# pyprob/pyprob

Measured on NVIDIA H100. Metric: ic_train_traces_per_sec, higher is better.
Workload: dtype f32

## Files before the change

pyprob_b200/csrc/net.cu:

```cuda
#include <vector>
#include <string.h>
#include <stdlib.h>
#include <stdint.h>

#include "common.cuh"
#include "gemm_simt.cuh"
#include "heads.cuh"
#include "tc_grouped.cuh"
#include "tc_lstm.cuh"
#include "tc_cluster.cuh"
#include "tc_persist.cuh"
#include "obs_mlp.cuh"

using gemm::Problem;

struct HImg {
  float* k_hi = nullptr; float* k_lo = nullptr; float* mn_hi = nullptr; float* mn_lo = nullptr;
  int64_t kb = 0;
};

struct WImg {
  int64_t k_hi = 0, k_lo = 0, mn_hi = 0, mn_lo = 0;
  int kb = 0;
};
struct PackEntry {
  int64_t src_off;
  int rows, cols, ld, kb;
  int64_t k_hi, k_lo, mn_hi, mn_lo;
  int tile_start, pad_;
};

enum class ObsForm { fused, tensor_core, simt };

struct ppb_net {
  float* wimg = nullptr;
  int64_t wimg_floats = 0;
  std::vector<PackEntry> pack;
  PackEntry* d_pack = nullptr;
  int pack_tiles = 0;
  WImg w_ihE, w_hh;
  std::vector<WImg> w1, w2;
  ObsForm obs_form = ObsForm::simt;
  WImg w_obs[PPB_MAX_OBS][PPB_MAX_FF_LAYERS];
  WImg w_fin[PPB_MAX_FF_LAYERS];
  uint64_t slot_hash[10] = {0, 0, 0, 0, 0, 0, 0, 0, 0, 0};
  const void* slot_dev[10] = {nullptr, nullptr, nullptr, nullptr, nullptr, nullptr, nullptr, nullptr, nullptr, nullptr};
  void* h_blob[2] = {nullptr, nullptr};
  cudaEvent_t ev_blob[2] = {nullptr, nullptr};
  size_t blob_cap = 0;
  int blob_idx = 0;
  ppb_net_desc desc;
  std::vector<ppb_addr_desc> addrs;
  std::vector<int64_t> type_off;
  ppb_addr_desc* d_addrs = nullptr;
  int64_t* d_type_off = nullptr;
  int64_t arena_floats = 0;
  int I = 0;
  int dh_pad = 4;
  int out_pad = 4;
  bool fused_cell = true;
  float* whh_il = nullptr;
  int64_t whh_il_floats = 0;
  void* d_lstm_steps = nullptr;
  size_t lstm_steps_cap = 0;
  cudaStream_t side[2] = {nullptr, nullptr};
  cudaEvent_t fork_ev[16] = {nullptr, nullptr, nullptr, nullptr, nullptr, nullptr, nullptr, nullptr,
                             nullptr, nullptr, nullptr, nullptr, nullptr, nullptr, nullptr, nullptr};
  int fork_next = 0;
  int single_stream = 0;
  int pack_tiles_no_hh = 0;
  int host_graph = 1;
  cudaStream_t host_stream = nullptr;
  cudaGraphExec_t host_exec = nullptr;
  uint64_t host_key = 0;
  int host_seen = 0;
  float* host_hyper_dev = nullptr;
  void* host_state_dev = nullptr;
  float host_hyper[6] = {0, 0, 0, 0, 0, 0};
  int64_t host_step_dev = -1;
  char* host_pin = nullptr;
  int64_t host_pin_cap = 0;
  Problem* h_stage[2] = {nullptr, nullptr};
  cudaEvent_t ev_stage[2] = {nullptr, nullptr};
  size_t stage_cap = 0;
  int stage_idx = 0;
};

namespace {

inline int64_t align_up(int64_t x, int64_t a) { return (x + a - 1) / a * a; }

struct Ws {
  float* obs_act[PPB_MAX_OBS][PPB_MAX_FF_LAYERS];
  float* obs_cat; float* fin_act[PPB_MAX_FF_LAYERS]; float* obs_emb;
  float* p_obs; float* emb_cat; float* p_step; float* w_smp_t; float* smp_emb;
  float* gates; float* c; float* h; float* hid; float* out_raw; float* row_lp; float* d_out;
  float* loss_acc;
  float* d_hid; float* dh; float* dh_rec; float* dc; float* d_pobs; float* d_pstep; float* d_smp; float* d_embcat;
  float* d_obs_emb; float* d_fin_act[PPB_MAX_FF_LAYERS]; float* d_obs_cat; float* d_obs_act[PPB_MAX_OBS][PPB_MAX_FF_LAYERS];
  Problem* problems;
  int64_t max_problems;
  int64_t total_bytes;
};

struct Dims {
  int B, R, T, NS, G;
};

Ws carve(const ppb_net* net, Dims d, void* base) {
  const ppb_net_desc& D = net->desc;
  Ws w;
  memset(&w, 0, sizeof(w));
  char* p = (char*)base;
  int64_t off = 0;
  auto take = [&](int64_t floats) {
    float* r = (float*)(p + off);
    off += align_up(floats * 4, 256);
    return r;
  };
  const int H = D.lstm_dim, E = D.obs_dim, S = D.sample_dim, C2 = 2 * (D.type_dim + D.addr_dim);
  for (int j = 0; j < D.num_obs; ++j)
    for (int l = 0; l + 1 < D.obs_ff[j].num_layers; ++l) w.obs_act[j][l] = take((int64_t)d.B * D.obs_ff[j].layers[l].out_dim);
  w.obs_cat = take((int64_t)d.B * E);
  for (int l = 0; l + 1 < D.obs_final.num_layers; ++l) w.fin_act[l] = take((int64_t)d.B * D.obs_final.layers[l].out_dim);
  w.obs_emb = take((int64_t)d.B * E);
  w.p_obs = take((int64_t)d.B * 4 * H);
  w.emb_cat = take((int64_t)d.NS * C2);
  w.p_step = take((int64_t)d.NS * 4 * H);
  w.w_smp_t = take((int64_t)S * 4 * H);
  w.smp_emb = take((int64_t)d.R * S);
  w.gates = take((int64_t)d.R * 4 * H);
  w.c = take((int64_t)d.R * H);
  w.h = take((int64_t)d.R * H);
  w.hid = take((int64_t)d.R * net->dh_pad);
  w.out_raw = take((int64_t)d.R * net->out_pad);
  w.row_lp = take(d.R);
  w.d_out = take((int64_t)d.R * net->out_pad);
  w.loss_acc = take(64);
  w.d_hid = take((int64_t)d.R * net->dh_pad);
  w.dh = take((int64_t)d.R * H);
  w.dh_rec = take((int64_t)d.R * H);
  w.dc = take((int64_t)d.R * H);
  w.d_pobs = take((int64_t)d.B * 4 * H);
  w.d_smp = take((int64_t)d.R * S);
  w.d_embcat = take((int64_t)d.NS * C2);
  w.d_pstep = take((int64_t)d.NS * 4 * H);
  w.d_obs_emb = take((int64_t)d.B * E);
  for (int l = 0; l + 1 < D.obs_final.num_layers; ++l) w.d_fin_act[l] = take((int64_t)d.B * D.obs_final.layers[l].out_dim);
  w.d_obs_cat = take((int64_t)d.B * E);
  for (int j = 0; j < D.num_obs; ++j)
    for (int l = 0; l + 1 < D.obs_ff[j].num_layers; ++l) w.d_obs_act[j][l] = take((int64_t)d.B * D.obs_ff[j].layers[l].out_dim);
  w.max_problems = 2 * (64 + 4LL * PPB_MAX_OBS * PPB_MAX_FF_LAYERS + 8LL * d.G + 4LL * d.T);
  w.problems = (Problem*)take(w.max_problems * (int64_t)(sizeof(Problem) / 4));
  w.total_bytes = off;
  return w;
}

inline float* dgates_ptr(const Ws& w, void* base) { return (float*)((char*)base + w.total_bytes); }
inline int64_t dgates_bytes(const ppb_net* net, Dims d) { return align_up((int64_t)d.R * 4 * net->desc.lstm_dim * 4, 256); }

struct Builder {
  std::vector<Problem> probs;
  std::vector<gemm::Phase> phases;
  void begin() { gemm::Phase ph; ph.first = (int)probs.size(); phases.push_back(ph); }
  void add(Problem p) {
    gemm::Phase& ph = phases.back();
    p.tiles_m = (p.M + gemm::BM - 1) / gemm::BM;
    p.tiles_n = (p.N + gemm::BN - 1) / gemm::BN;
    p.tile_start = ph.tiles;
    if (p.M <= 0 || p.N <= 0) return;
    ph.tiles += p.tiles_m * p.tiles_n;
    ph.count += 1;
    probs.push_back(p);
  }
};

inline Problem P0() {
  Problem p;
  memset(&p, 0, sizeof(p));
  p.alpha = 1.0f;
  return p;
}

inline Problem linear_fwd(const float* X, int64_t ldx, const float* W, int64_t ldw, const float* b, float* Y,
                          int64_t ldy, int M, int N, int K, int flags) {
  Problem p = P0();
  p.A = X; p.sam = ldx; p.sak = 1;
  p.B = W; p.sbn = ldw; p.sbk = 1;
  p.C = Y; p.ldc = ldy; p.bias = b;
  p.M = M; p.N = N; p.K = K; p.flags = flags;
  return p;
}
inline Problem linear_dx(const float* dY, int64_t lddy, const float* W, int64_t ldw, float* dX, int64_t lddx, int M,
                         int N, int K, int flags) {
  Problem p = P0();
  p.A = dY; p.sam = lddy; p.sak = 1;
  p.B = W; p.sbn = 1; p.sbk = ldw;
  p.C = dX; p.ldc = lddx;
  p.M = M; p.N = K; p.K = N; p.flags = flags;
  return p;
}
inline Problem linear_dw(const float* dY, int64_t lddy, const float* X, int64_t ldx, float* dW, int64_t ldw, int M,
                         int N, int K) {
  Problem p = P0();
  p.A = dY; p.sam = 1; p.sak = lddy;
  p.B = X; p.sbn = 1; p.sbk = ldx;
  p.C = dW; p.ldc = ldw;
  p.M = N; p.N = K; p.K = M; p.flags = gemm::kAccumulate;
  return p;
}

inline uint64_t fnv1a(const void* data, size_t n, uint64_t h = 1469598103934665603ULL) {
  const unsigned char* p = (const unsigned char*)data;
  for (size_t i = 0; i < n; ++i) { h ^= p[i]; h *= 1099511628211ULL; }
  return h;
}

int upload_cached(ppb_net* net, int slot, const void* src, size_t bytes, void* dev, cudaStream_t st) {
  if (bytes == 0) return PPB_OK;
  uint64_t h = fnv1a(src, bytes, 1469598103934665603ULL ^ (uint64_t)bytes);
  if (net->slot_hash[slot] == h && net->slot_dev[slot] == dev) return PPB_OK;
// ... 384 lines not shown
  NllArgs A;
  float* loss_acc; float* loss_out; int* status_out;
  struct State { float local; int bad; };
  using RowIn = NllRowIn;
  __device__ __forceinline__ RowIn load(int64_t row) const { return nll_row_in(A, (int)row); }
  __device__ __forceinline__ void row(State& s, const RowIn& in, const float* x, int64_t row, int lane) const {
    nll_row(A, in, x, (int)row, lane, s.local, s.bad);
  }
  __device__ __forceinline__ void finish(const State& s, int lane) const {
    nll_finish(s.local, s.bad, lane, A.inv_batch, gridDim.x, loss_acc, loss_out, status_out);
  }
};

__global__ void __launch_bounds__(256) k_head_nll(const float* __restrict__ out_raw, NllArgs A, int R,
                                                   float* __restrict__ loss_acc, float* __restrict__ loss_out,
                                                   int* __restrict__ status_out) {
  ppb_pdl_trigger();
  ppb_pdl_wait();
  const int lane = threadIdx.x & 31;
  const int warp = (blockIdx.x * blockDim.x + threadIdx.x) >> 5, nwarps = (gridDim.x * blockDim.x) >> 5;
  float local = 0.0f;
  int bad = 0;
  for (int row = warp; row < R; row += nwarps) nll_row(A, out_raw + (int64_t)row * A.out_pad, row, lane, local, bad);
  nll_finish(local, bad, lane, A.inv_batch, gridDim.x, loss_acc, loss_out, status_out);
}

__global__ void __launch_bounds__(256, 4) k_head_out_nll(const float* __restrict__ arena, const float* __restrict__ hid_hi,
                                                       const float* __restrict__ hid_lo, int64_t hid_kb,
                                                       const int* __restrict__ step_row0, const int* __restrict__ step_nrows,
                                                       int rows_per_block, NllArgs A, float* __restrict__ out_raw,
                                                       float* __restrict__ loss_acc, float* __restrict__ loss_out,
                                                       int* __restrict__ status_out) {
  ppb_pdl_trigger();
  extern __shared__ float sm_head[];
  const int seg = blockIdx.y, warp = threadIdx.x >> 5, lane = threadIdx.x & 31;
  const ppb_addr_desc a = A.addrs[A.step_addr[seg]];
  const int Hh = a.head_hidden, O = a.head_out, Hh4 = (Hh + 3) & ~3;
  const int pitch = ((Hh4 >> 2) & 1) ? Hh4 : Hh4 + 4;
  float* w2s = sm_head;
  float* b2s = w2s + (size_t)O * pitch;
  float* hrow = b2s + ((O + 3) & ~3) + (size_t)warp * (Hh4 + 128);
  float* xout = hrow + Hh4;
  const int r0 = step_row0[seg] + blockIdx.x * rows_per_block;
  int r1 = r0 + rows_per_block;
  const int seg_end = step_row0[seg] + step_nrows[seg];
  const int seg_end_pad = step_row0[seg] + ((step_nrows[seg] + 127) & ~127);
  if (r1 > seg_end_pad) r1 = seg_end_pad;
  const bool any = r0 < r1 && r0 < seg_end;
  if (any) {
    const float* w2 = arena + a.w2_off;
    for (int i = threadIdx.x; i < O * pitch; i += blockDim.x) {
      const int o = i / pitch, k = i - o * pitch;
      w2s[i] = (k < Hh) ? __ldg(w2 + (int64_t)o * Hh + k) : 0.0f;
    }
    for (int o = threadIdx.x; o < O; o += blockDim.x) b2s[o] = __ldg(arena + a.b2_off + o);
  }
  ppb_pdl_wait();
  __syncthreads();
  float local = 0.0f;
  int bad = 0;
  for (int row = r0 + warp; row < r1; row += 8) {
    if (row >= seg_end) {
      nll_row(A, xout, row, lane, local, bad);
      continue;
    }
    for (int k = lane; k < Hh4; k += 32) {
      float v = 0.0f;
      if (k < Hh) {
        const int64_t off = tc::packed_offset(row, k, hid_kb);
        v = __ldg(hid_hi + off) + (hid_lo ? __ldg(hid_lo + off) : 0.0f);
      }
      hrow[k] = v;
    }
    __syncwarp();
    for (int o0 = 0; o0 < O; o0 += 32) {
      const int o = o0 + lane;
      const float4* wr = reinterpret_cast<const float4*>(w2s + (size_t)(o < O ? o : 0) * pitch);
      const float4* hr = reinterpret_cast<const float4*>(hrow);
      float acc[4] = {0.f, 0.f, 0.f, 0.f};
#pragma unroll 4
      for (int k4 = 0; k4 < (Hh4 >> 2); ++k4) {
        const float4 h4 = hr[k4], w4 = wr[k4];
        acc[0] = fmaf(h4.x, w4.x, acc[0]);
        acc[1] = fmaf(h4.y, w4.y, acc[1]);
        acc[2] = fmaf(h4.z, w4.z, acc[2]);
        acc[3] = fmaf(h4.w, w4.w, acc[3]);
      }
      if (o < O) {
        const float y = ((acc[0] + acc[1]) + (acc[2] + acc[3])) + b2s[o];
        xout[o] = y;
        if (out_raw) out_raw[(int64_t)row * A.out_pad + o] = y;
      }
    }
    __syncwarp();
    nll_row(A, xout, row, lane, local, bad);
    __syncwarp();
  }
  nll_finish(local, bad, lane, A.inv_batch, gridDim.x * gridDim.y, loss_acc, loss_out, status_out);
}

__device__ __forceinline__ float cell_bwd_unit(float ig, float fg, float gg, float og, float cn, float cp, float dht,
                                               float dc_next, float (&dv)[4]) {
  const float tc_ = ppb_cell_tanh(cn);
  const float dct = dc_next + dht * og * (1.0f - tc_ * tc_);
  dv[0] = dct * gg * ig * (1.0f - ig);
  dv[1] = dct * cp * fg * (1.0f - fg);
  dv[2] = dct * ig * (1.0f - gg * gg);
  dv[3] = dht * tc_ * og * (1.0f - og);
  return dct;
}

__device__ __forceinline__ void img_store_gates(const HImg& img, int64_t row, int j, int64_t gate_stride, const float (&v)[4]) {
  const int64_t ok = tc::packed_offset(row, j, img.kb), omn = tc::packed_offset_mn(row, j, img.kb);
#pragma unroll
  for (int q = 0; q < 4; ++q) {
    float hi, lo;
    tc::split_tf32(v[q], hi, lo);
    img.k_hi[ok + q * gate_stride] = hi;
    if (img.k_lo) img.k_lo[ok + q * gate_stride] = lo;
    if (img.mn_hi) {
      img.mn_hi[omn + q * gate_stride] = hi;
      if (img.mn_lo) img.mn_lo[omn + q * gate_stride] = lo;
    }
  }
}

struct CellBwdT1Epi {
  const float* gates; const float* c; const int* row_trace;
  float* dgates; HImg pimg; int H;
  __device__ __forceinline__ void cells(int64_t row, int j0, const float (&dh)[4]) const {
    const int tr = __ldg(row_trace + row);
    const int64_t gate_stride = (int64_t)(H >> 5) * tc::kTileFloats;
    float gv[4][4], cv[4];
#pragma unroll
    for (int u = 0; u < 4; ++u) {
      const int j = min(j0 + 32 * u, H - 1);
#pragma unroll
      for (int q = 0; q < 4; ++q) gv[u][q] = __ldg(gates + row * 4 * H + q * H + j);
      cv[u] = __ldg(c + row * H + j);
    }
#pragma unroll
    for (int u = 0; u < 4; ++u) {
      const int j = j0 + 32 * u;
      if (j >= H) continue;
      float dv[4] = {0.f, 0.f, 0.f, 0.f};
      if (tr >= 0) cell_bwd_unit(gv[u][0], gv[u][1], gv[u][2], gv[u][3], cv[u], 0.0f, dh[u], 0.0f, dv);
#pragma unroll
      for (int q = 0; q < 4; ++q) dgates[row * 4 * H + q * H + j] = dv[q];
      if (tr >= 0) img_store_gates(pimg, tr, j, gate_stride, dv);
    }
  }
};

template <bool FINAL>
__global__ void __launch_bounds__(256, FINAL ? 4 : 8) k_cell_bwd(const float* __restrict__ gates, const float* __restrict__ c,
                                                   const float* __restrict__ dh, const float* __restrict__ dh_rec,
                                                   float* __restrict__ dc, float* __restrict__ dgates,
                                                   float* __restrict__ d_pobs, const int* __restrict__ row_prev,
                                                   const int* __restrict__ row_next, const int* __restrict__ row_trace,
                                                   HImg gimg, int row0, int n_rows, int H, int t, HImg pimg) {
  ppb_pdl_trigger();
  ppb_pdl_wait();
  const int64_t total = (int64_t)n_rows * H;
  const int64_t gate_stride = (int64_t)(H >> 5) * tc::kTileFloats;
  const bool h32 = (H & 31) == 0;
  for (int64_t e = (int64_t)blockIdx.x * blockDim.x + threadIdx.x; e < total; e += (int64_t)gridDim.x * blockDim.x) {
    const int i = (int)(e / H), j = (int)(e - (int64_t)i * H);
    const int row = row0 + i;
    const int tr = __ldg(row_trace + row);
    const int64_t rH = (int64_t)row * H + j;
    float* dgr = dgates + (int64_t)row * 4 * H + j;
    float dv[4] = {0.f, 0.f, 0.f, 0.f};
    if (tr >= 0) {
      const int nx = __ldg(row_next + row);
      const float* g = gates + (int64_t)row * 4 * H + j;
      const float ig = g[0], fg = g[H], gg = g[2 * H], og = g[3 * H];
      const float cn = c[rH];
      const float cp = (t > 0) ? c[(int64_t)__ldg(row_prev + row) * H + j] : 0.0f;
      const bool has_next = nx >= 0;
      const float dht = dh[rH] + (has_next ? dh_rec[rH] : 0.0f);
      const float dct = cell_bwd_unit(ig, fg, gg, og, cn, cp, dht, has_next ? dc[(int64_t)nx * H + j] : 0.0f, dv);
      if (dc) dc[rH] = dct * fg;
      float* dp = d_pobs + (int64_t)tr * 4 * H + j;
      float tot[4];
#pragma unroll
      for (int q = 0; q < 4; ++q) {
        tot[q] = has_next ? dp[q * H] + dv[q] : dv[q];
        dp[q * H] = tot[q];
      }
      if (FINAL && pimg.k_hi) img_store_gates(pimg, tr, j, gate_stride, tot);
    }
#pragma unroll
    for (int q = 0; q < 4; ++q) dgr[q * H] = dv[q];
    if (gimg.k_hi) {
      if (h32) {
        img_store_gates(gimg, row, j, gate_stride, dv);
      } else {
#pragma unroll
        for (int q = 0; q < 4; ++q)
          tcg::img_store(gimg.k_hi, gimg.k_lo, gimg.mn_hi, gimg.mn_lo, row, q * H + j, gimg.kb, dv[q]);
      }
    }
  }
}

__global__ void __launch_bounds__(256) k_step_colsum(const float* __restrict__ dgates, const int* __restrict__ step_row0,
                                                      const int* __restrict__ step_nrows, int H4,
                                                      float* __restrict__ d_pstep) {
  __shared__ float part[8][33];
  const int st = blockIdx.y;
  const int r0 = step_row0[st], n = step_nrows[st];
  const int lane = threadIdx.x & 31, slice = threadIdx.x >> 5;
  const int col = blockIdx.x * 32 + lane;
  float s = 0.0f;
  if (col < H4)
    for (int r = slice; r < n; r += 8) s += dgates[(int64_t)(r0 + r) * H4 + col];
  part[slice][lane] = s;
  __syncthreads();
  if (slice == 0 && col < H4) {
    float t = 0.0f;
#pragma unroll
    for (int k = 0; k < 8; ++k) t += part[k][lane];
    d_pstep[(int64_t)st * H4 + col] = t;
  }
}

__global__ void __launch_bounds__(128) k_smp_bwd(const float* __restrict__ dgates, const float* __restrict__ w_smp_t,
                                                  const float* __restrict__ smp_emb, const float* __restrict__ values,
                                                  const int* __restrict__ row_step, const int* __restrict__ step_prev,
                                                  const int* __restrict__ row_prev,
                                                  const ppb_addr_desc* __restrict__ addrs, int R, int H4, int S,
                                                  float* __restrict__ grad) {
  int warp = (blockIdx.x * blockDim.x + threadIdx.x) >> 5, lane = threadIdx.x & 31;
  int nwarps = (gridDim.x * blockDim.x) >> 5;
  for (int row = warp; row < R; row += nwarps) {
    int pa = step_prev[row_step[row]];
    if (pa < 0) continue;
    const ppb_addr_desc& a = addrs[pa];
    float x = values[row_prev[row]];
    for (int j = 0; j < S; ++j) {
      float s = 0.0f;
      for (int col = lane; col < H4; col += 32) s = fmaf(dgates[(int64_t)row * H4 + col], w_smp_t[(int64_t)j * H4 + col], s);
      s = ppb_warp_sum(s);
      if (lane == 0 && smp_emb[(int64_t)row * S + j] > 0.0f && s != 0.0f) {
        atomicAdd(grad + a.smp_b_off + j, s);
        if (a.family == PPB_FAMILY_CATEGORICAL) {
          int cidx = (int)x;
          if (cidx >= 0 && cidx < a.smp_in) atomicAdd(grad + a.smp_w_off + (int64_t)j * a.smp_in + cidx, s);
        } else {
          atomicAdd(grad + a.smp_w_off + (int64_t)j * a.smp_in, s * x);
        }
      }
    }
  }
}

__global__ void __launch_bounds__(128) k_smp_bwd_seg(const float* __restrict__ dgates, const float* __restrict__ w_smp_t,
                                                      const float* __restrict__ smp_emb, const float* __restrict__ values,
                                                      const int* __restrict__ step_prev, const int* __restrict__ step_row0,
                                                      const int* __restrict__ step_nrows, const int* __restrict__ row_prev,
                                                      const ppb_addr_desc* __restrict__ addrs, int H4, int S,
                                                      int rows_per_block, float* __restrict__ grad) {
  __shared__ float acc_b[8];
  __shared__ float acc_w[8][heads::CMAX];
  const int st = blockIdx.y;
  const int pa = step_prev[st];
  if (pa < 0) return;
  const int seg0 = step_row0[st], r0 = seg0 + blockIdx.x * rows_per_block;
  int r1 = r0 + rows_per_block;
  if (r1 > seg0 + step_nrows[st]) r1 = seg0 + step_nrows[st];
  if (r0 >= r1) return;
  const ppb_addr_desc a = addrs[pa];
  const bool is_cat = a.family == PPB_FAMILY_CATEGORICAL;
  const int width = is_cat ? a.smp_in : 1;
  for (int i = threadIdx.x; i < 8 * heads::CMAX; i += blockDim.x) (&acc_w[0][0])[i] = 0.0f;
  if (threadIdx.x < 8) acc_b[threadIdx.x] = 0.0f;
  __syncthreads();
  const int warp = threadIdx.x >> 5, lane = threadIdx.x & 31;
  for (int row = r0 + warp; row < r1; row += 4) {
    float s[8];
#pragma unroll
    for (int j = 0; j < 8; ++j) s[j] = 0.0f;
    for (int col = lane; col < H4; col += 32) {
      const float d = dgates[(int64_t)row * H4 + col];
#pragma unroll
      for (int j = 0; j < 8; ++j)
        if (j < S) s[j] = fmaf(d, __ldg(w_smp_t + (int64_t)j * H4 + col), s[j]);
    }
#pragma unroll
    for (int j = 0; j < 8; ++j)
      if (j < S) s[j] = ppb_warp_sum(s[j]);
    if (lane == 0) {
      const float x = values[row_prev[row]];
      const int cidx = (int)x;
#pragma unroll
      for (int j = 0; j < 8; ++j) {
        if (j < S && smp_emb[(int64_t)row * S + j] > 0.0f && s[j] != 0.0f) {
          atomicAdd(&acc_b[j], s[j]);
          if (is_cat) { if (cidx >= 0 && cidx < a.smp_in) atomicAdd(&acc_w[j][cidx], s[j]); }
          else atomicAdd(&acc_w[j][0], s[j] * x);
        }
      }
    }
  }
  __syncthreads();
  for (int i = threadIdx.x; i < S * (width + 1); i += blockDim.x) {
// ... 130 lines not shown
    }
    for (int j = 0; j < S; ++j)
      if (acc[j] != 0.0f) atomicAdd(dw_ih + (int64_t)col * I + E + j, acc[j]);
  }
}

__global__ void k_bias_grad(const float* __restrict__ d_pstep, int NS, int H4, float* __restrict__ db_ih,
                            float* __restrict__ db_hh) {
  for (int col = blockIdx.x * blockDim.x + threadIdx.x; col < H4; col += gridDim.x * blockDim.x) {
    float s = 0.0f;
    for (int st = 0; st < NS; ++st) s += d_pstep[(int64_t)st * H4 + col];
    db_ih[col] += s;
    db_hh[col] += s;
  }
}
__global__ void k_embed_scatter(const float* __restrict__ d_embcat, const ppb_addr_desc* __restrict__ addrs,
                                const int64_t* __restrict__ type_off, const int* __restrict__ step_addr,
                                const int* __restrict__ step_prev, int n_steps, int td, int ad,
                                float* __restrict__ grad) {
  int C2 = 2 * (td + ad);
  for (int64_t e = (int64_t)blockIdx.x * blockDim.x + threadIdx.x; e < (int64_t)n_steps * C2;
       e += (int64_t)gridDim.x * blockDim.x) {
    int st = (int)(e / C2), j = (int)(e % C2);
    int which = j < (td + ad) ? step_prev[st] : step_addr[st];
    int jj = j < (td + ad) ? j : j - (td + ad);
    if (which < 0) continue;
    const ppb_addr_desc& a = addrs[which];
    float v = d_embcat[e];
    if (v == 0.0f) continue;
    if (jj < td) atomicAdd(grad + type_off[a.type_id] + jj, v);
    else atomicAdd(grad + a.addr_emb_off + (jj - td), v);
  }
}
__global__ void __launch_bounds__(256) k_colsum_gather(const float* __restrict__ dY, int64_t ld,
                                                        const int* __restrict__ m_gather, int M, int N,
                                                        float* __restrict__ db) {
  __shared__ float part[8][33];
  const int lane = threadIdx.x & 31, slice = threadIdx.x >> 5;
  const int n = blockIdx.x * 32 + lane;
  float s = 0.0f;
  if (n < N)
    for (int m = blockIdx.y * 8 + slice; m < M; m += 8 * gridDim.y) {
      int64_t pm = m_gather ? m_gather[m] : m;
      s += dY[pm * ld + n];
    }
  part[slice][lane] = s;
  __syncthreads();
  if (slice == 0 && n < N) {
    float t = 0.0f;
#pragma unroll
    for (int k = 0; k < 8; ++k) t += part[k][lane];
    if (t != 0.0f) atomicAdd(db + n, t);
  }
}
__global__ void k_scale(float* __restrict__ x, int64_t n, float a) {
  for (int64_t i = (int64_t)blockIdx.x * blockDim.x + threadIdx.x; i < n; i += (int64_t)gridDim.x * blockDim.x) x[i] *= a;
}

__global__ void k_add_row_bias(float* __restrict__ p, const float* __restrict__ b, int64_t n, int H4) {
  for (int64_t i = (int64_t)blockIdx.x * blockDim.x + threadIdx.x; i < n; i += (int64_t)gridDim.x * blockDim.x) p[i] += b[i % H4];
}
__global__ void k_mask_nonpos(float* __restrict__ d, const float* __restrict__ y, int64_t n) {
  for (int64_t i = (int64_t)blockIdx.x * blockDim.x + threadIdx.x; i < n; i += (int64_t)gridDim.x * blockDim.x)
    if (!(y[i] > 0.0f)) d[i] = 0.0f;
}

inline int ew_grid(int64_t n, int threads = 256) { return ppb_grid_for(n, threads, 1); }

Dims dims_of(const ppb_batch* b) {
  Dims d; d.B = b->n_traces; d.R = b->n_rows; d.T = b->t_max; d.NS = b->n_steps; d.G = b->n_groups;
  return d;
}

int check_batch(const ppb_net* net, const ppb_batch* b) {
  PPB_CHECK_ARG(net && b, "null net or batch");
  PPB_CHECK_ARG(b->n_traces > 0 && b->n_rows > 0 && b->t_max > 0 && b->n_steps > 0 && b->n_groups > 0, "empty batch");
  PPB_CHECK_ARG(b->row_off_host && b->group_addr_host && b->group_start_host, "missing host arrays");
  PPB_CHECK_ARG(b->row_off_host[0] == 0 && b->row_off_host[b->t_max] == b->n_rows, "row_off inconsistent");
  for (int g = 0; g < b->n_groups; ++g)
    PPB_CHECK_ARG(b->group_addr_host[g] >= 0 && b->group_addr_host[g] < (int)net->addrs.size(), "address id out of range");
  return PPB_OK;
}

}

#include "net_tc.inc"

extern "C" {

int ppb_net_create(ppb_net** out, const ppb_net_desc* d) {
  PPB_CHECK_ARG(out && d, "null argument");
  PPB_CHECK_ARG(d->lstm_dim > 0 && d->obs_dim > 0 && d->sample_dim > 0 && d->sample_dim <= 8, "bad dims");
  PPB_CHECK_ARG(d->num_obs > 0 && d->num_obs <= PPB_MAX_OBS, "bad observable count");
  PPB_CHECK_ARG(d->mixture_k > 0 && d->mixture_k <= heads::KMAX, "mixture components must be in [1,32]");
  ppb_net* n = new ppb_net();
  n->desc = *d;
  n->I = d->obs_dim + d->sample_dim + 2 * (d->type_dim + d->addr_dim);
  const char* fc = getenv("PPB_FUSED_CELL");
  n->fused_cell = !(fc && fc[0] == '0');
  const char* hg = getenv("PPB_HOST_STEP_GRAPH");
  n->host_graph = (hg && hg[0] == '0') ? 0 : 1;
  const char* ss = getenv("PPB_SINGLE_STREAM");
  n->single_stream = (ss && ss[0] == '1') ? 1 : 0;
  for (int i = 0; i < 16; ++i) PPB_CUDA(cudaEventCreateWithFlags(&n->fork_ev[i], cudaEventDisableTiming));
  if (!n->single_stream)
    for (int i = 0; i < 2; ++i) PPB_CUDA(cudaStreamCreateWithFlags(&n->side[i], cudaStreamNonBlocking));
  *out = n;
  return PPB_OK;
}

int ppb_net_set_tables(ppb_net* net, const ppb_addr_desc* addrs, int32_t n_addrs, const int64_t* type_off,
                       int32_t n_types, int64_t arena_floats) {
  PPB_CHECK_ARG(net && addrs && type_off && n_addrs > 0 && n_types > 0, "bad arguments");
  net->addrs.assign(addrs, addrs + n_addrs);
  net->type_off.assign(type_off, type_off + n_types);
  net->arena_floats = arena_floats;
  int dh = 4, op = 4;
  for (auto& a : net->addrs) {
    PPB_CHECK_ARG(a.family >= 0 && a.family <= PPB_FAMILY_BERNOULLI, "unknown family");
    PPB_CHECK_ARG(a.family != PPB_FAMILY_CATEGORICAL || (a.num_categories > 0 && a.num_categories <= heads::CMAX),
                  "categorical head: 1..128 categories supported");
    PPB_CHECK_ARG(a.family != PPB_FAMILY_BERNOULLI || (a.head_out == 1 && a.smp_in == 1 && a.num_categories == 0),
                  "bernoulli head: head_out = 1, smp_in = 1, num_categories = 0");
    PPB_CHECK_ARG(a.type_id >= 0 && a.type_id < n_types, "type id out of range");
    if (a.head_hidden > dh) dh = a.head_hidden;
    if (a.head_out > op) op = a.head_out;
  }
  net->dh_pad = (int)align_up(dh, 4);
  net->out_pad = (int)align_up(op, 4);
  if (net->d_addrs) cudaFree(net->d_addrs);
  if (net->d_type_off) cudaFree(net->d_type_off);
  PPB_CUDA(cudaMalloc((void**)&net->d_addrs, sizeof(ppb_addr_desc) * n_addrs));
  PPB_CUDA(cudaMalloc((void**)&net->d_type_off, sizeof(int64_t) * n_types));
  PPB_CUDA(cudaMemcpy(net->d_addrs, addrs, sizeof(ppb_addr_desc) * n_addrs, cudaMemcpyHostToDevice));
  PPB_CUDA(cudaMemcpy(net->d_type_off, type_off, sizeof(int64_t) * n_types, cudaMemcpyHostToDevice));
  return build_weight_images(net);
}

int ppb_net_destroy(ppb_net* net) {
  if (!net) return PPB_OK;
  if (net->d_addrs) cudaFree(net->d_addrs);
  if (net->d_type_off) cudaFree(net->d_type_off);
  for (int i = 0; i < 2; ++i) {
    if (net->h_stage[i]) cudaFreeHost(net->h_stage[i]);
    if (net->ev_stage[i]) cudaEventDestroy(net->ev_stage[i]);
    if (net->h_blob[i]) cudaFreeHost(net->h_blob[i]);
    if (net->ev_blob[i]) cudaEventDestroy(net->ev_blob[i]);
  }
  for (int i = 0; i < 2; ++i) if (net->side[i]) cudaStreamDestroy(net->side[i]);
  for (int i = 0; i < 16; ++i) if (net->fork_ev[i]) cudaEventDestroy(net->fork_ev[i]);
  if (net->wimg) cudaFree(net->wimg);
  if (net->d_pack) cudaFree(net->d_pack);
  if (net->whh_il) cudaFree(net->whh_il);
  if (net->d_lstm_steps) cudaFree(net->d_lstm_steps);
  if (net->host_exec) cudaGraphExecDestroy(net->host_exec);
  if (net->host_stream) cudaStreamDestroy(net->host_stream);
  if (net->host_hyper_dev) cudaFree(net->host_hyper_dev);
  if (net->host_state_dev) cudaFree(net->host_state_dev);
  if (net->host_pin) cudaFreeHost(net->host_pin);
  delete net;
  return PPB_OK;
}

int64_t ppb_ic_workspace_bytes(const ppb_net* net, int32_t n_traces, int32_t n_rows, int32_t t_max, int32_t n_steps,
                               int32_t n_groups) {
  if (!net || n_traces <= 0 || n_rows <= 0) return -1;
  Dims d; d.B = n_traces; d.R = n_rows; d.T = t_max; d.NS = n_steps; d.G = n_groups;
  return simt_region_bytes(net, d) + carve_tc(net, d, nullptr).total_bytes + 1024;
}

int ppb_ic_loss_forward(ppb_net* net, const float* arena, const ppb_batch* b, void* workspace,
                        int64_t workspace_bytes, int precision, float* loss_out, int32_t* status_out,
                        float* row_lp_out, int want_grad, void* stream) {
  int rc = check_batch(net, b);
  if (rc) return rc;
  PPB_CHECK_ARG(arena && workspace, "null arena/workspace");
  PPB_CHECK_ARG(!net->addrs.empty(), "address tables not set");
  PPB_CHECK_ARG(precision >= 0 && precision <= 2, "unknown precision mode");
  const ppb_net_desc& D = net->desc;
  Dims d = dims_of(b);
  PPB_CHECK_ARG(workspace_bytes >= ppb_ic_workspace_bytes(net, d.B, d.R, d.T, d.NS, d.G), "workspace too small");
  cudaStream_t st = (cudaStream_t)stream;
  if (precision != PPB_PREC_FP32_SIMT)
    return tc_loss_forward(net, arena, b, workspace, precision, loss_out, status_out, row_lp_out, want_grad, st);
  PPB_CHECK_ARG(b->row_align == 1, "the SIMT path needs a batch encoded with row_align = 1");
  Ws w = carve(net, d, workspace);
  const int H = D.lstm_dim, H4 = 4 * H, E = D.obs_dim, S = D.sample_dim, I = net->I;
  const int C2 = 2 * (D.type_dim + D.addr_dim);

  Builder bl;
  obs_fp32_plan_fwd(bl, D, arena, b->obs, d.B, w, w.obs_emb);
  const int ph_obs0 = 0;
  const int ph_p = (int)bl.phases.size();
  bl.begin();
  bl.add(linear_fwd(w.obs_emb, E, arena + D.w_ih_off, I, nullptr, w.p_obs, H4, d.B, H4, E, 0));
  bl.add(linear_fwd(w.emb_cat, C2, arena + D.w_ih_off + E + S, I, arena + D.b_ih_off, w.p_step, H4, d.NS, H4, C2, 0));
  const int ph_rec0 = (int)bl.phases.size();
  for (int t = 1; t < d.T; ++t) {
    bl.begin();
    int r0 = b->row_off_host[t], n = b->row_off_host[t + 1] - r0, rp = b->row_off_host[t - 1];
    bl.add(linear_fwd(w.h + (int64_t)rp * H, H, arena + D.w_hh_off, H, nullptr, w.gates + (int64_t)r0 * H4, H4, n, H4, H, 0));
  }
  const int ph_h1 = (int)bl.phases.size();
  bl.begin();
  for (int g = 0; g < d.G; ++g) {
    const ppb_addr_desc& a = net->addrs[b->group_addr_host[g]];
    int s0 = b->group_start_host[g], cnt = b->group_start_host[g + 1] - s0;
    Problem p = linear_fwd(w.h, H, arena + a.w1_off, H, arena + a.b1_off, w.hid, net->dh_pad, cnt, a.head_hidden, H, gemm::kRelu);
    p.m_gather = b->head_rows + s0;
    bl.add(p);
  }
  const int ph_h2 = (int)bl.phases.size();
  bl.begin();
  for (int g = 0; g < d.G; ++g) {
    const ppb_addr_desc& a = net->addrs[b->group_addr_host[g]];
    int s0 = b->group_start_host[g], cnt = b->group_start_host[g + 1] - s0;
    Problem p = linear_fwd(w.hid, net->dh_pad, arena + a.w2_off, a.head_hidden, arena + a.b2_off, w.out_raw, net->out_pad, cnt, a.head_out, a.head_hidden, 0);
    p.m_gather = b->head_rows + s0;
    bl.add(p);
  }
  rc = upload_and_get(net, bl, w.problems, w.max_problems / 2, st, 0);
  if (rc) return rc;

  PPB_CUDA(cudaMemsetAsync(w.loss_acc, 0, 256, st));
  for (int l = ph_obs0; l < ph_p; ++l) { rc = run_phase(bl.phases[l], w.problems, st); if (rc) return rc; }
  k_step_embed<<<ew_grid((int64_t)d.NS * C2), 256, 0, st>>>(arena, net->d_addrs, net->d_type_off, b->step_addr,
                                                            b->step_prev_addr, d.NS, D.type_dim, D.addr_dim, w.emb_cat);
  PPB_LAUNCH_CHECK();
  k_wsmp_transpose<<<ew_grid(S * H4), 256, 0, st>>>(arena + D.w_ih_off, I, E, S, H4, w.w_smp_t);
  PPB_LAUNCH_CHECK();
  k_smp_embed<<<ew_grid((int64_t)d.R * S), 256, 0, st>>>(arena, net->d_addrs, b->row_step, b->step_prev_addr,
                                                         b->row_prev, b->values, d.R, S, w.smp_emb);
  PPB_LAUNCH_CHECK();
  rc = run_phase(bl.phases[ph_p], w.problems, st, &bl);
  if (rc) return rc;
  k_add_row_bias<<<ew_grid((int64_t)d.NS * H4), 256, 0, st>>>(w.p_step, arena + D.b_hh_off, (int64_t)d.NS * H4, H4);
  PPB_LAUNCH_CHECK();
  for (int t = 0; t < d.T; ++t) {
    int r0 = b->row_off_host[t], n = b->row_off_host[t + 1] - r0;
    if (t > 0) { rc = run_phase(bl.phases[ph_rec0 + t - 1], w.problems, st, &bl); if (rc) return rc; }
    k_cell_fwd<<<ew_grid((int64_t)n * H), 256, 0, st>>>(w.gates, w.p_obs, w.p_step, w.w_smp_t, w.smp_emb, b->row_step,
                                                       b->row_prev, b->row_trace, w.c, w.h, HImg(), r0, n, H, S, t);
    PPB_LAUNCH_CHECK();
  }
  rc = run_phase(bl.phases[ph_h1], w.problems, st); if (rc) return rc;
  rc = run_phase(bl.phases[ph_h2], w.problems, st); if (rc) return rc;
  {
    NllArgs na;
    na.addrs = net->d_addrs; na.row_step = b->row_step; na.step_addr = b->step_addr;
    na.values = b->values; na.prior0 = b->prior0; na.prior1 = b->prior1; na.row_trace = b->row_trace;
    na.K = D.mixture_k; na.inv_batch = 1.0f / (float)d.B;
    na.row_lp = row_lp_out ? row_lp_out : w.row_lp; na.d_out = want_grad ? w.d_out : nullptr; na.out_pad = net->out_pad;
    na.dimg = HImg();
    k_head_nll<<<ew_grid((int64_t)d.R * 32, 256), 256, 0, st>>>(w.out_raw, na, d.R, w.loss_acc, loss_out, status_out);
  }
  PPB_LAUNCH_CHECK();
  return PPB_OK;
}

int ppb_ic_loss_backward(ppb_net* net, const float* arena, float* grad, const ppb_batch* b, void* workspace,
                         int64_t workspace_bytes, int precision, float grad_scale, void* stream) {
  int rc = check_batch(net, b);
  if (rc) return rc;
  PPB_CHECK_ARG(arena && grad && workspace, "null arena/grad/workspace");
  const ppb_net_desc& D = net->desc;
  Dims d = dims_of(b);
  PPB_CHECK_ARG(workspace_bytes >= ppb_ic_workspace_bytes(net, d.B, d.R, d.T, d.NS, d.G), "workspace too small");
  cudaStream_t st = (cudaStream_t)stream;
  if (precision != PPB_PREC_FP32_SIMT) return tc_loss_backward(net, arena, grad, b, workspace, precision, grad_scale, st);
  Ws w = carve(net, d, workspace);
  float* dgates = dgates_ptr(w, workspace);
  const int H = D.lstm_dim, H4 = 4 * H, E = D.obs_dim, S = D.sample_dim, I = net->I;
  const int C2 = 2 * (D.type_dim + D.addr_dim);

  if (grad_scale != 1.0f) {
    k_scale<<<ew_grid((int64_t)d.R * net->out_pad), 256, 0, st>>>(w.d_out, (int64_t)d.R * net->out_pad, grad_scale);
    PPB_LAUNCH_CHECK();
  }

  Builder bl;
  const int ph_dhid = 0;
  bl.begin();
  for (int g = 0; g < d.G; ++g) {
    const ppb_addr_desc& a = net->addrs[b->group_addr_host[g]];
    int s0 = b->group_start_host[g], cnt = b->group_start_host[g + 1] - s0;
    Problem p = linear_dx(w.d_out, net->out_pad, arena + a.w2_off, a.head_hidden, w.d_hid, net->dh_pad, cnt, a.head_out, a.head_hidden, gemm::kMaskAux);
    p.aux = w.hid; p.ld_aux = net->dh_pad; p.m_gather = b->head_rows + s0;
    bl.add(p);
  }
  const int ph_hw = 1;
  bl.begin();
  for (int g = 0; g < d.G; ++g) {
    const ppb_addr_desc& a = net->addrs[b->group_addr_host[g]];
    int s0 = b->group_start_host[g], cnt = b->group_start_host[g + 1] - s0;
    Problem p2 = linear_dw(w.d_out, net->out_pad, w.hid, net->dh_pad, grad + a.w2_off, a.head_hidden, cnt, a.head_out, a.head_hidden);
    p2.ka_gather = b->head_rows + s0; p2.kb_gather = b->head_rows + s0;
    bl.add(p2);
    Problem p1 = linear_dw(w.d_hid, net->dh_pad, w.h, H, grad + a.w1_off, H, cnt, a.head_hidden, H);
    p1.ka_gather = b->head_rows + s0; p1.kb_gather = b->head_rows + s0;
    bl.add(p1);
    Problem px = linear_dx(w.d_hid, net->dh_pad, arena + a.w1_off, H, w.dh, H, cnt, a.head_hidden, H, 0);
    px.m_gather = b->head_rows + s0;
    bl.add(px);
  }
  const int ph_rec0 = 2;
  for (int t = d.T - 1; t >= 1; --t) {
// ... 669 lines not shown
```

pyprob_b200/csrc/net_tc.inc:

```
extern unsigned long long* g_trace;
extern int g_trace_launch;

namespace {

inline int64_t img_floats(int64_t rows, int64_t cols) {
  return ((rows + 127) / 128) * ((cols + 31) / 32) * tc::kTileFloats;
}

__global__ void __launch_bounds__(256) k_pack_table(const float* __restrict__ arena, const PackEntry* __restrict__ tab,
                                                     int n_entries, float* __restrict__ wimg) {
  int tile = blockIdx.x;
  int lo = 0, hi = n_entries - 1;
  while (lo < hi) {
    int mid = (lo + hi + 1) >> 1;
    if (tab[mid].tile_start <= tile) lo = mid; else hi = mid - 1;
  }
  const PackEntry e = tab[lo];
  const int rt = tile - e.tile_start;
  const float* src = arena + e.src_off;
  for (int q = threadIdx.x + blockIdx.y * blockDim.x; q < 128 * e.kb * 8; q += blockDim.x * gridDim.y) {
    int c16 = q & 7, t = q >> 3;
    int cb = t % e.kb, r = t / e.kb;
    int row = rt * 128 + r, k0 = cb * 32 + c16 * 4;
    float h[4], l[4];
// ... 719 lines not shown

  TcBuilder tb;
  std::vector<std::vector<int>> addr_chunks(net->addrs.size());
  std::vector<int> hh_a, hh_b;
  for (int s = 0; s < d.NS; ++s) {
    int r0 = b->step_row0_host[s], np = pad128(b->step_nrows_host[s]);
    for (int q = 0; q < np; q += 32) {
      addr_chunks[b->step_addr_host[s]].push_back(r0 + q);
      if (b->step_t_host[s] > 0) { hh_a.push_back(r0 + q); hh_b.push_back(b->step_prev_row0_host[s] + q); }
    }
  }
  std::vector<int> chunk_off(net->addrs.size(), -1);
  for (size_t a = 0; a < net->addrs.size(); ++a) {
    if (addr_chunks[a].empty()) continue;
    chunk_off[a] = (int)tb.ints.size();
    tb.ints.insert(tb.ints.end(), addr_chunks[a].begin(), addr_chunks[a].end());
  }
  const int hh_a_off = (int)tb.ints.size();
  tb.ints.insert(tb.ints.end(), hh_a.begin(), hh_a.end());
  const int hh_b_off = (int)tb.ints.size();
  tb.ints.insert(tb.ints.end(), hh_b.begin(), hh_b.end());
  PPB_CHECK_ARG((int64_t)tb.ints.size() <= t.max_ints, "chunk list overflow");

  const int ph_dhid = 0;
  tb.begin();
  for (int s = 0; s < d.NS; ++s) {
    int aid = b->step_addr_host[s];
    const ppb_addr_desc& a = net->addrs[aid];
    tcg::Problem p = TP0();
    p.a = op_k(t.d_out.k_hi, t.d_out.k_lo, okb, b->step_row0_host[s], 0);
    p.b = wmn(net, net->w2[aid]);
    p.M = pad128(b->step_nrows_host[s]); p.N = a.head_hidden; p.K = a.head_out;
    p.flags = tcg::kMaskImg;
    p.mask_hi = t.hid.k_hi;
    p.c = w.d_hid + (int64_t)b->step_row0_host[s] * net->dh_pad; p.ldc = net->dh_pad;
    p.o_k_hi = t.d_hid.k_hi; p.o_k_lo = t.d_hid.k_lo; p.o_mn_hi = t.d_hid.mn_hi; p.o_mn_lo = t.d_hid.mn_lo;
    p.o_kb = dhkb; p.o_row0 = b->step_row0_host[s]; p.o_col0 = 0;
    tb.add(p);
  }
  const int ph_hw = (int)tb.phases.size();
  tb.begin();
  for (int s = 0; s < d.NS; ++s) {
    int aid = b->step_addr_host[s];
    const ppb_addr_desc& a = net->addrs[aid];
    tcg::Problem p = TP0();
    p.a = op_k(t.d_hid.k_hi, t.d_hid.k_lo, dhkb, b->step_row0_host[s], 0);
    p.b = wmn(net, net->w1[aid]);
    p.M = pad128(b->step_nrows_host[s]); p.N = H; p.K = a.head_hidden;
    p.c = w.dh + (int64_t)b->step_row0_host[s] * H; p.ldc = H;
    p.o_row0 = b->step_row0_host[s];
    tb.add(p);
  }
  const int ph_headw = (int)tb.phases.size();
  tb.begin();
  int headw_tiles = 0;
  for (size_t aid = 0; aid < net->addrs.size(); ++aid) {
    if (chunk_off[aid] < 0) continue;
    const ppb_addr_desc& a = net->addrs[aid];
    headw_tiles += ((a.head_out + 127) / 128) * ((a.head_hidden + 127) / 128) + ((a.head_hidden + 127) / 128) * ((H + 127) / 128);
  }
  for (size_t aid = 0; aid < net->addrs.size(); ++aid) {
    if (chunk_off[aid] < 0) continue;
    const ppb_addr_desc& a = net->addrs[aid];
    const int* kr = t.ints + chunk_off[aid];
    int nch = (int)addr_chunks[aid].size();
    tcg::Problem p2 = TP0();
    p2.a = op_mn(t.d_out.mn_hi, t.d_out.mn_lo, okb, 0, 0, kr);
    p2.b = op_mn(t.hid.mn_hi, t.hid.mn_lo, dhkb, 0, 0, kr);
    p2.M = a.head_out; p2.N = a.head_hidden; p2.K = 32 * nch;
    p2.c = grad + a.w2_off; p2.ldc = a.head_hidden; p2.flags = tcg::kAccumulate;
    p2.k_splits = pick_splits(p2.M, p2.N, p2.K, headw_tiles);
    tb.add(p2);
    tcg::Problem p1 = TP0();
    p1.a = op_mn(t.d_hid.mn_hi, t.d_hid.mn_lo, dhkb, 0, 0, kr);
    p1.b = op_mn(t.h.mn_hi, t.h.mn_lo, hkb, 0, 0, kr);
    p1.M = a.head_hidden; p1.N = H; p1.K = 32 * nch;
    p1.c = grad + a.w1_off; p1.ldc = H; p1.flags = tcg::kAccumulate;
    p1.k_splits = pick_splits(p1.M, p1.N, p1.K, headw_tiles);
    tb.add(p1);
  }
  std::vector<int> ph_rec(d.T, -1);
  {
    int st1 = d.NS;
    for (int tt = d.T - 1; tt >= 1; --tt) {
      int st0 = st1;
      while (st0 > 0 && b->step_t_host[st0 - 1] == tt) --st0;
      ph_rec[tt] = (int)tb.phases.size();
      tb.begin();
      for (int s = st0; s < st1; ++s) {
        tcg::Problem p = TP0();
        p.a = op_k(t.dgates.k_hi, t.dgates.k_lo, gkb, b->step_row0_host[s], 0);
        p.b = wmn(net, net->w_hh);
        p.M = pad128(b->step_nrows_host[s]); p.N = H; p.K = H4;
        p.c = w.dh_rec + (int64_t)b->step_prev_row0_host[s] * H; p.ldc = H;
        tb.add(p);
      }
      {
        gemm::Phase& ph = tb.phases.back();
        int rows = 0;
        for (int i = 0; i < ph.count; ++i) rows += tb.probs[ph.first + i].M;
        const int splits = pick_splits(rows, H, H4);
        ph.tiles = 0;
        for (int i = 0; i < ph.count; ++i) {
          tcg::Problem& p = tb.probs[ph.first + i];
          p.k_splits = splits;
          p.tile_start = ph.tiles;
          ph.tiles += p.tiles_m * p.tiles_n * splits;
        }
      }
      st1 = st0;
    }
  }

  const int ph_lstm_w = (int)tb.phases.size();
  tb.begin();
  if (!hh_a.empty()) {
    tcg::Problem p = TP0();
    p.a = op_mn(t.dgates.mn_hi, t.dgates.mn_lo, gkb, 0, 0, t.ints + hh_a_off);
    p.b = op_mn(t.h.mn_hi, t.h.mn_lo, hkb, 0, 0, t.ints + hh_b_off);
    p.M = H4; p.N = H; p.K = 32 * (int)hh_a.size();
    p.c = grad + D.w_hh_off; p.ldc = H; p.flags = tcg::kAccumulate;
    p.k_splits = pick_splits(p.M, p.N, p.K);
    tb.add(p);
  }
  {
    tcg::Problem p = TP0();
    p.a = op_mn(t.dpobs.mn_hi, t.dpobs.mn_lo, gkb, 0, 0);
    p.b = op_mn(t.obs_emb.mn_hi, t.obs_emb.mn_lo, (int)t.obs_emb.kb, 0, 0);
    p.M = H4; p.N = E; p.K = pad128(d.B);
    p.c = grad + D.w_ih_off; p.ldc = I; p.flags = tcg::kAccumulate;
    p.k_splits = pick_splits(p.M, p.N, p.K);
    tb.add(p);
    tcg::Problem q = TP0();
    q.a = op_k(t.dpobs.k_hi, t.dpobs.k_lo, gkb, 0, 0);
    q.b = wmn(net, net->w_ihE);
    q.M = d.B; q.N = E; q.K = H4;
    q.c = w.d_obs_emb; q.ldc = E;
    q.k_splits = pick_splits(q.M, q.N, q.K);
    tb.add(q);
  }
  ObsStep os;
  rc = obs_plan_bwd(net, arena, grad, b, w, t.obs, tb, os, st);
  if (rc) return rc;
  PPB_CHECK_ARG((int64_t)tb.probs.size() <= t.max_probs / 2, "tensor-core problem list overflow");
  tcg::Problem* tprobs = t.probs + t.max_probs / 2;
  rc = upload_cached(net, 3, tb.probs.data(), tb.probs.size() * sizeof(tcg::Problem), tprobs, st);
  if (rc) return rc;
  rc = upload_cached(net, 4, tb.ints.data(), tb.ints.size() * sizeof(int), t.ints, st);
  if (rc) return rc;

  cudaStream_t s1, s2;
  rc = side_stream(net, 0, st, &s1); if (rc) return rc;
  rc = side_stream(net, 1, st, &s2); if (rc) return rc;
  if (d.T > 1) PPB_CUDA(cudaMemsetAsync(w.dh_rec, 0, (size_t)b->row_off_host[d.T - 1] * H * sizeof(float), st));
  PPB_CUDA(cudaMemsetAsync(w.d_pstep, 0, (size_t)((const char*)(w.d_obs_emb + (int64_t)d.B * E) - (const char*)w.d_pstep), st));
  rc = run_tc_phase_auto(tb.phases[ph_dhid], tprobs, precision, st, 2, tb); if (rc) return rc;
  static const bool fuse_pack_on = [] { const char* e = getenv("PPB_FUSE_PACK"); return !(e && e[0] == '0'); }();
  const bool dpobs_fused = fuse_pack_on && (d.B & 127) == 0 && t.dgates.k_hi != nullptr;
  bool dpobs_packed = false;
  const int cs_cell = (d.T == 1 && dpobs_fused) ? phase_cluster(tb.phases[ph_hw], tb, true) : 1;
  if (cs_cell > 1) {
    CellBwdT1Epi re;
    re.gates = w.gates; re.c = w.c; re.row_trace = b->row_trace; re.dgates = dgates; re.pimg = t.dpobs; re.H = H;
    rc = run_tc_phase_cluster<4>(cs_cell, tb.phases[ph_hw], tprobs, precision, st, re); if (rc) return rc;
    dpobs_packed = true;
  } else {
    rc = run_tc_phase_auto(tb.phases[ph_hw], tprobs, precision, st, 0, tb); if (rc) return rc;
    const HImg gimg = d.T > 1 ? t.dgates : HImg();
    float* const dc = d.T > 1 ? w.dc : nullptr;
    for (int tt = d.T - 1; tt >= 0; --tt) {
      int r0 = b->row_off_host[tt], n = b->row_off_host[tt + 1] - r0;
      if (tt + 1 < d.T) { rc = run_tc_phase(tb.phases[ph_rec[tt + 1]], tprobs, precision, st, 1, &tb); if (rc) return rc; }
      if (tt == 0 && dpobs_fused) {
        PPB_CUDA(ppb_launch(k_cell_bwd<true>, dim3(ew_grid((int64_t)n * H)), dim3(256), 0, st, 1, 0, w.gates, w.c, w.dh, w.dh_rec,
                            dc, dgates, w.d_pobs, b->row_prev, b->row_next, b->row_trace, gimg, r0, n, H, tt, t.dpobs));
        dpobs_packed = true;
      } else {
        PPB_CUDA(ppb_launch(k_cell_bwd<false>, dim3(ew_grid((int64_t)n * H)), dim3(256), 0, st, 1, 0, w.gates, w.c, w.dh, w.dh_rec,
                            dc, dgates, w.d_pobs, b->row_prev, b->row_next, b->row_trace, gimg, r0, n, H, tt, HImg()));
      }
      PPB_LAUNCH_CHECK();
    }
  }
  rc = stream_after(net, st, s1); if (rc) return rc;
  rc = run_tc_phase(tb.phases[ph_headw], tprobs, precision, s1, 1); if (rc) return rc;
  {
    const int cb = (net->dh_pad + 31) / 32 + (net->out_pad + 31) / 32;
    int max_rows = 0;
    for (int g = 0; g < d.G; ++g) max_rows = b->group_start_host[g + 1] - b->group_start_host[g] > max_rows ? b->group_start_host[g + 1] - b->group_start_host[g] : max_rows;
    int zs = PPB_NUM_SMS / (cb * d.G);
    const int zmax = (max_rows + 63) / 64;
    zs = zs > zmax ? zmax : zs;
    zs = zs < 1 ? 1 : zs;
    k_head_bias_grad<<<dim3(cb, d.G, zs), 256, 0, s1>>>(w.d_out, net->out_pad, w.d_hid, net->dh_pad, b->head_rows, b->group_start,
                                                         b->group_addr, net->d_addrs, grad);
    PPB_LAUNCH_CHECK();
  }
  rc = stream_after(net, st, s2); if (rc) return rc;
  const bool one_pass = S <= 4 && H4 <= 2048;
  int max_rows = 0;
  for (int s = 0; s < d.NS; ++s) max_rows = b->step_nrows_host[s] > max_rows ? b->step_nrows_host[s] : max_rows;
  if (one_pass) {
    int slab = (d.R + 2 * PPB_NUM_SMS - 1) / (2 * PPB_NUM_SMS);
    slab = slab < 4 ? 4 : (slab > kRedSlab ? kRedSlab : slab);
    const dim3 g((max_rows + slab - 1) / slab, d.NS);
    const float* wt = d.T > 1 ? w.w_smp_t : w.p_step;
    if (H4 <= 1024)
      k_dgates_reduce<4><<<g, 256, 0, s2>>>(dgates, wt, w.smp_emb, b->values, b->step_prev_addr, b->step_row0, b->step_nrows,
                                            b->row_prev, net->d_addrs, H4, S, I, E, w.d_pstep, grad, D.w_ih_off, slab);
    else
      k_dgates_reduce<8><<<g, 256, 0, s2>>>(dgates, wt, w.smp_emb, b->values, b->step_prev_addr, b->step_row0, b->step_nrows,
                                            b->row_prev, net->d_addrs, H4, S, I, E, w.d_pstep, grad, D.w_ih_off, slab);
    PPB_LAUNCH_CHECK();
  } else {
    dim3 g((H4 + 31) / 32, d.NS);
    k_step_colsum<<<g, 256, 0, s2>>>(dgates, b->step_row0, b->step_nrows, H4, w.d_pstep);
    PPB_LAUNCH_CHECK();
  }
  {
    const int jbs = (C2 + 31) / 32;
    int zsplit = PPB_NUM_SMS / 2 / (jbs * d.NS);
    zsplit = zsplit < 1 ? 1 : (zsplit > 16 ? 16 : zsplit);
    const int nx = jbs * d.NS * zsplit;
    const int nw = (int)(((int64_t)H4 * C2 + H4 + 255) / 256);
    k_pstep_bwd<<<nx + nw, 256, 0, s2>>>(w.d_pstep, arena + D.w_ih_off, w.emb_cat, net->d_addrs, net->d_type_off, b->step_addr,
                                         b->step_prev_addr, d.NS, H4, I, E + S, D.type_dim, D.addr_dim, zsplit, nx, grad,
                                         D.w_ih_off, D.b_ih_off, D.b_hh_off);
    PPB_LAUNCH_CHECK();
  }
  if (d.T > 1 && !one_pass) {
    const int slab = 64;
    k_smp_bwd_seg<<<dim3((max_rows + slab - 1) / slab, d.NS), 128, 0, s2>>>(dgates, w.w_smp_t, w.smp_emb, b->values,
                                                                           b->step_prev_addr, b->step_row0, b->step_nrows,
                                                                           b->row_prev, net->d_addrs, H4, S, slab, grad);
    PPB_LAUNCH_CHECK();
    int rpb = 1024;
    dim3 g((H4 + 255) / 256, (d.R + rpb - 1) / rpb);
    k_wsmp_grad<<<g, 256, 0, s2>>>(dgates, w.smp_emb, d.R, H4, S, I, E, grad + D.w_ih_off, rpb);
    PPB_LAUNCH_CHECK();
  }
  if (!dpobs_packed) {
    PPB_CUDA(ppb_launch(k_pack_rows, dim3(dim3((d.B + 127) / 128, 64)), dim3(256), 0, st, 1, 0, w.d_pobs, d.B, H4, H4, t.dpobs));
    PPB_LAUNCH_CHECK();
  }
  rc = run_tc_phase(tb.phases[ph_lstm_w], tprobs, precision, st, 1, &tb); if (rc) return rc;
  rc = obs_bwd(net, arena, grad, b, w, t.obs, tb, tprobs, os, precision, st); if (rc) return rc;
  rc = stream_after(net, s1, st); if (rc) return rc;
  return stream_after(net, s2, st);
}

}
```

Measured before the change: 1.586 million.

## Add SIMT head d_hid kernel and move gradient zeroing to side stream

Adds a custom warp-per-row kernel for the head hidden-gradient computation. It stages the output weight in shared memory, applies the ReLU mask and writes both the dense and packed tensor-core images. This kernel replaces the tensor-core grouped phase when the weights fit and the phase would otherwise be clustered. The memsets of dh_rec and the gradient region now run on a side stream and are joined lazily before their first consumer, so they overlap the head backward. This adds event synchronization complexity, and the scalar FMA path may be slower than tensor cores for large heads.

```diff
diff --git a/pyprob_b200/csrc/net.cu b/pyprob_b200/csrc/net.cu
--- a/pyprob_b200/csrc/net.cu
+++ b/pyprob_b200/csrc/net.cu
@@ -67,6 +67,7 @@
   cudaEvent_t fork_ev[16] = {nullptr, nullptr, nullptr, nullptr, nullptr, nullptr, nullptr, nullptr,
                              nullptr, nullptr, nullptr, nullptr, nullptr, nullptr, nullptr, nullptr};
   int fork_next = 0;
+  cudaEvent_t ev_zero = nullptr;
   int single_stream = 0;
   int pack_tiles_no_hh = 0;
   int host_graph = 1;
@@ -757,6 +758,71 @@
   }
 };
 
+constexpr int kDhidWarps = 4;
+constexpr int kDhidMaxBlocks = 12;
+__global__ void __launch_bounds__(32 * kDhidWarps) k_head_dhid(const float* __restrict__ arena,
+                                                              const ppb_addr_desc* __restrict__ addrs,
+                                                              const int* __restrict__ step_addr,
+                                                              const int* __restrict__ step_row0,
+                                                              const int* __restrict__ step_nrows,
+                                                              const float* __restrict__ d_out, int out_pad,
+                                                              const float* __restrict__ hid_k_hi, float* __restrict__ d_hid,
+                                                              int dh_pad, HImg img) {
+  ppb_pdl_trigger();
+  extern __shared__ float w2s[];
+  const int seg = blockIdx.y, warp = threadIdx.x >> 5, lane = threadIdx.x & 31;
+  const int nrows = __ldg(step_nrows + seg);
+  const int i0 = blockIdx.x * kDhidWarps;
+  if (i0 >= ((nrows + 127) & ~127)) return;
+  const ppb_addr_desc& a = addrs[__ldg(step_addr + seg)];
+  const int Hh = a.head_hidden, O = a.head_out;
+  if (i0 < nrows) {
+    const float* const w2 = arena + a.w2_off;
+    for (int e = threadIdx.x; e < O * Hh; e += blockDim.x) w2s[e] = __ldg(w2 + e);
+  }
+  ppb_pdl_wait();
+  __syncthreads();
+  const int i = i0 + warp;
+  if (i >= ((nrows + 127) & ~127)) return;
+  const int64_t row = (int64_t)__ldg(step_row0 + seg) + i;
+  const int nblk = (int)img.kb;
+  if (i >= nrows) {
+    for (int c = lane; c < nblk * 32; c += 32) {
+      if (c < dh_pad) d_hid[row * dh_pad + c] = 0.0f;
+      tcg::img_store(img.k_hi, img.k_lo, img.mn_hi, img.mn_lo, row, c, img.kb, 0.0f);
+    }
+    return;
+  }
+  const float* const dor = d_out + row * out_pad;
+  for (int c0 = 0; c0 < nblk; c0 += kDhidMaxBlocks) {
+    float acc[kDhidMaxBlocks];
+#pragma unroll
+    for (int q = 0; q < kDhidMaxBlocks; ++q) acc[q] = 0.0f;
+    for (int o0 = 0; o0 < O; o0 += 32) {
+      const float dv = o0 + lane < O ? dor[o0 + lane] : 0.0f;
+      const int on = O - o0 < 32 ? O - o0 : 32;
+      for (int oo = 0; oo < on; ++oo) {
+        const float d = __shfl_sync(0xffffffffu, dv, oo);
+        const float* const wr = w2s + (o0 + oo) * Hh;
+#pragma unroll
+        for (int q = 0; q < kDhidMaxBlocks; ++q) {
+          const int c = (c0 + q) * 32 + lane;
+          if (c < Hh) acc[q] = fmaf(d, wr[c], acc[q]);
+        }
+      }
+    }
+#pragma unroll
+    for (int q = 0; q < kDhidMaxBlocks; ++q) {
+      const int c = (c0 + q) * 32 + lane;
+      if (c0 + q >= nblk) break;
+      float x = 0.0f;
+      if (c < Hh && __ldg(hid_k_hi + tc::packed_offset(row, c, img.kb)) > 0.0f) x = acc[q];
+      if (c < dh_pad) d_hid[row * dh_pad + c] = x;
+      tcg::img_store(img.k_hi, img.k_lo, img.mn_hi, img.mn_lo, row, c, img.kb, x);
+    }
+  }
+}
+
 template <bool FINAL>
 __global__ void __launch_bounds__(256, FINAL ? 4 : 8) k_cell_bwd(const float* __restrict__ gates, const float* __restrict__ c,
                                                    const float* __restrict__ dh, const float* __restrict__ dh_rec,
@@ -1193,6 +1259,7 @@
   if (net->wimg) cudaFree(net->wimg);
   if (net->d_pack) cudaFree(net->d_pack);
   if (net->whh_il) cudaFree(net->whh_il);
+  if (net->ev_zero) cudaEventDestroy(net->ev_zero);
   if (net->d_lstm_steps) cudaFree(net->d_lstm_steps);
   if (net->host_exec) cudaGraphExecDestroy(net->host_exec);
   if (net->host_stream) cudaStreamDestroy(net->host_stream);
diff --git a/pyprob_b200/csrc/net_tc.inc b/pyprob_b200/csrc/net_tc.inc
--- a/pyprob_b200/csrc/net_tc.inc
+++ b/pyprob_b200/csrc/net_tc.inc
@@ -895,9 +895,38 @@
   cudaStream_t s1, s2;
   rc = side_stream(net, 0, st, &s1); if (rc) return rc;
   rc = side_stream(net, 1, st, &s2); if (rc) return rc;
-  if (d.T > 1) PPB_CUDA(cudaMemsetAsync(w.dh_rec, 0, (size_t)b->row_off_host[d.T - 1] * H * sizeof(float), st));
-  PPB_CUDA(cudaMemsetAsync(w.d_pstep, 0, (size_t)((const char*)(w.d_obs_emb + (int64_t)d.B * E) - (const char*)w.d_pstep), st));
-  rc = run_tc_phase_auto(tb.phases[ph_dhid], tprobs, precision, st, 2, tb); if (rc) return rc;
+  rc = stream_after(net, st, s2); if (rc) return rc;
+  if (d.T > 1) PPB_CUDA(cudaMemsetAsync(w.dh_rec, 0, (size_t)b->row_off_host[d.T - 1] * H * sizeof(float), s2));
+  PPB_CUDA(cudaMemsetAsync(w.d_pstep, 0, (size_t)((const char*)(w.d_obs_emb + (int64_t)d.B * E) - (const char*)w.d_pstep), s2));
+  if (!net->ev_zero) PPB_CUDA(cudaEventCreateWithFlags(&net->ev_zero, cudaEventDisableTiming));
+  PPB_CUDA(cudaEventRecord(net->ev_zero, s2));
+  bool zero_joined = false;
+  auto join_zero = [&]() -> int {
+    if (!zero_joined) { PPB_CUDA(cudaStreamWaitEvent(st, net->ev_zero, 0)); zero_joined = true; }
+    return PPB_OK;
+  };
+  size_t dhid_smem = 0;
+  int dhid_pad = 0;
+  for (int s = 0; s < d.NS; ++s) {
+    const ppb_addr_desc& a = net->addrs[b->step_addr_host[s]];
+    const size_t f = (size_t)a.head_out * a.head_hidden * sizeof(float);
+    dhid_smem = f > dhid_smem ? f : dhid_smem;
+    dhid_pad = pad128(b->step_nrows_host[s]) > dhid_pad ? pad128(b->step_nrows_host[s]) : dhid_pad;
+  }
+  if (dhid_smem <= 100 * 1024 && phase_cluster(tb.phases[ph_dhid], tb, true) > 1) {
+    static bool attr = false;
+    if (!attr) {
+      PPB_CUDA(cudaFuncSetAttribute(k_head_dhid, cudaFuncAttributeMaxDynamicSharedMemorySize, 100 * 1024));
+      attr = true;
+    }
+    PPB_CUDA(ppb_launch(k_head_dhid, dim3(dhid_pad / kDhidWarps, d.NS), dim3(32 * kDhidWarps), dhid_smem, st, 1, 0, arena,
+                        (const ppb_addr_desc*)net->d_addrs, (const int*)b->step_addr, (const int*)b->step_row0,
+                        (const int*)b->step_nrows, (const float*)w.d_out, net->out_pad, (const float*)t.hid.k_hi, w.d_hid,
+                        net->dh_pad, t.d_hid));
+    PPB_LAUNCH_CHECK();
+  } else {
+    rc = run_tc_phase_auto(tb.phases[ph_dhid], tprobs, precision, st, 2, tb); if (rc) return rc;
+  }
   static const bool fuse_pack_on = [] { const char* e = getenv("PPB_FUSE_PACK"); return !(e && e[0] == '0'); }();
   const bool dpobs_fused = fuse_pack_on && (d.B & 127) == 0 && t.dgates.k_hi != nullptr;
   bool dpobs_packed = false;
@@ -913,7 +942,10 @@
     float* const dc = d.T > 1 ? w.dc : nullptr;
     for (int tt = d.T - 1; tt >= 0; --tt) {
       int r0 = b->row_off_host[tt], n = b->row_off_host[tt + 1] - r0;
-      if (tt + 1 < d.T) { rc = run_tc_phase(tb.phases[ph_rec[tt + 1]], tprobs, precision, st, 1, &tb); if (rc) return rc; }
+      if (tt + 1 < d.T) {
+        rc = join_zero(); if (rc) return rc;
+        rc = run_tc_phase(tb.phases[ph_rec[tt + 1]], tprobs, precision, st, 1, &tb); if (rc) return rc;
+      }
       if (tt == 0 && dpobs_fused) {
         PPB_CUDA(ppb_launch(k_cell_bwd<true>, dim3(ew_grid((int64_t)n * H)), dim3(256), 0, st, 1, 0, w.gates, w.c, w.dh, w.dh_rec,
                             dc, dgates, w.d_pobs, b->row_prev, b->row_next, b->row_trace, gimg, r0, n, H, tt, t.dpobs));
@@ -986,6 +1018,7 @@
     PPB_CUDA(ppb_launch(k_pack_rows, dim3(dim3((d.B + 127) / 128, 64)), dim3(256), 0, st, 1, 0, w.d_pobs, d.B, H4, H4, t.dpobs));
     PPB_LAUNCH_CHECK();
   }
+  rc = join_zero(); if (rc) return rc;
   rc = run_tc_phase(tb.phases[ph_lstm_w], tprobs, precision, st, 1, &tb); if (rc) return rc;
   rc = obs_bwd(net, arena, grad, b, w, t.obs, tb, tprobs, os, precision, st); if (rc) return rc;
   rc = stream_after(net, s1, st); if (rc) return rc;
```

New measurement: 1.624 million, median of 6. 1.02x the previous value.
